# orange-vertex/depthmapX

Hardware: AMD Instinct MI355X
Metric: grid cells/sec for VISPREP makeGraph + VGA global on N×N grid (higher is better)
Workload: dtype f64

## Files before the change

### depthmapx_amd/csrc/api/makegraph.hip

```cpp

typedef void (*mk_kernel_t)(const MakeGraphParams*);
#ifndef DMX_MK_WPE
#define DMX_MK_WPE 5
#endif
#define MKK(PROF, FIXED, COUNT, MAXD, FAR) makegraph_kernel<DMX_MK_WPE, PROF, FIXED, COUNT, MAXD, FAR>
static mk_kernel_t mk_kernel(bool fixed, bool count, bool maxd, bool far) {
    if (count) {
        if (!fixed || maxd) return MKK(false, false, true, false, false);
        return far ? MKK(false, true, true, false, true) : MKK(false, true, true, false, false);
    }
    if (verbose()) {
        if (!fixed || maxd) return MKK(true, false, false, false, false);
        return far ? MKK(true, true, false, false, true) : MKK(true, true, false, false, false);
    }
    if (!fixed) return MKK(false, false, false, false, false);
    if (maxd) return far ? MKK(false, true, false, true, true) : MKK(false, true, false, true, false);
    return far ? MKK(false, true, false, false, true) : MKK(false, true, false, false, false);
}
#undef MKK

static int mk_sqrt_err(dmx_ctx* ctx, long long nmax, double* err) {
    if (ctx->sqrt_err_nmax < nmax) {
        DevBuf<unsigned long long> e;
        HIPCHK(e.alloc(1));
// ... 163 lines not shown
            HIPCHK(hipMemsetAsync(ctx->counters.p + 4, 0, sizeof(int), ctx->stream));
            MakeGraphParams P;
            P.cols = h.cols(); P.rows = h.rows();
            P.spacing = h.spacing(); P.blx = h.bottom_left().x; P.bly = h.bottom_left().y;
            P.maxdist = maxdist;
            P.cellw = pm->d_cellw.p; P.segs = pm->d_segs.p; P.node_cell = pm->d_node_cell.p;
            P.sqrt_err = sqrt_err;
            P.node_begin = node_begin; P.node_end = node_end;
            P.work_counter = ctx->counters.p + 0;
            P.ctl = ctx->d_ctl;
            ctx->h_ctl->progress = 0;
            P.error = ctx->counters.p + 1;
            P.pool_cursor = (unsigned long long*)(ctx->counters.p + 2);
            P.pool_capacity = pool_cap; P.pool = g->pool.p;
            P.node_run_start = g->node_run_start.p; P.bin_nruns = g->bin_nruns.p; P.bin_count = g->bin_count.p;
            P.bin_dist = g->bin_dist.p; P.attrs = g->attrs.p;
            P.stageA = stA.p; P.stageB = stB.p; P.prefix = pref.p; P.runcnt = rcnt.p;
            P.capA = (int)capA; P.capB = (int)capB; P.gcap = gcap; P.bcap = bcap; P.dmax = D;
            P.bspill = bsp.p; P.bspill_flag = bspf.p; P.spill_cap = spill_cap;
            P.stats = ctx->stats.p;
            P.node_list = list_n < 0 ? nullptr : node_list.p;
            P.list_n = list_n < 0 ? 0 : list_n;
            P.fail_list = fail_list.p;
            P.fail_count = ctx->counters.p + 4;
            P.profile = verbose() ? 1 : 0;
            P.exact_moments = exact_pass ? 1 : 0;
            P.src_work = d_work;
            P.openh = openh.p; P.openh_n = openh_n;
            const bool sym_pass = fuse_sym && !sampling;
            P.sym_prefix = sym_pass ? g->sym_prefix.p : nullptr;
            P.sym_diff = sym_pass ? g->sym_diff.p : nullptr;
            P.sym_ho = sym_pass ? g->sym_ho.p : nullptr;
            P.spans = getenv("DMX_MK_NOSPAN") ? 0 : (getenv("DMX_MK_SPAN") ? std::max(1, atoi(getenv("DMX_MK_SPAN"))) : MK_SPAN_MIN);
            HIPCHK(hipEventRecord(ctx->ev0, ctx->stream));
            if (todo > 0) {
                HIPCHK(dP.alloc(1));
                HIPCHK(hipMemcpyAsync(dP.p, &P, sizeof(P), hipMemcpyHostToDevice, ctx->stream));
                hipLaunchKernelGGL(kern, dim3((unsigned)waves), dim3(64), lds, ctx->stream,
                                   (const MakeGraphParams*)dP.p);
                HIPCHK(hipGetLastError());
            }
            HIPCHK(hipEventRecord(ctx->ev1, ctx->stream));
            HIPCHK(wait_progress(ctx, DMX_PHASE_MAKEGRAPH, todo, 1));
            CANCEL_POINT(ctx);
            float ms = 0;
            HIPCHK(hipEventElapsedTime(&ms, ctx->ev0, ctx->ev1));
            kernel_s += ms * 1e-3;
            int hc[5] = {0, 0, 0, 0, 0};
            HIPCHK(copy_sync(ctx->stream, hc, ctx->counters.p, sizeof(hc), hipMemcpyDeviceToHost));
            const int err = hc[1], nfail = hc[4];
            VLOG("makegraph: attempt %d (%lld sources, gcap %d bcap %d spill %d capB %lld, occupancy %d): %.3f s, %d failed, "
                 "err %d\n", attempt, (long long)todo, gcap, bcap, spill_cap, (long long)capB, occ, ms * 1e-3, nfail, err);
            if (err & KERR_BIN_MISMATCH) return fail(DMX_ERR_STATE, "internal: whichbin outside octant");
            if (err & KERR_POOL_CAPACITY) {
                unsigned long long used = 0;
                std::memcpy(&used, &hc[2], 8);
                pool_cap = std::max<int64_t>(pool_cap * 2, (int64_t)used + 1024);
                pool_over = true;
                break;
            }
            if (nfail == 0) break;
            if (!sampling) {
                reruns += nfail;
                std::vector<int64_t> fl((size_t)nfail);
                HIPCHK(copy_sync(ctx->stream, fl.data(), fail_list.p, (size_t)nfail * 8, hipMemcpyDeviceToHost));
                mk_reruns.insert(mk_reruns.end(), fl.begin(), fl.end());
// ... 21 lines not shown
        HIPCHK(hipEventRecord(ctx->ev0, ctx->stream));
        if (n > 0 && !only) {
            hipLaunchKernelGGL(gridconn_kernel, dim3((unsigned)((n + 255) / 256)), dim3(256), 0, ctx->stream, h.rows(),
                               pm->d_node_cell.p + node_begin, n, g->node_run_start.p, g->bin_nruns.p, g->pool.p,
                               g->gridconn.p);
            HIPCHK(hipGetLastError());
            hipLaunchKernelGGL(node_nruns_kernel, dim3((unsigned)((n + 255) / 256)), dim3(256), 0, ctx->stream,
                               g->bin_nruns.p, n, g->node_nruns.p);
            HIPCHK(hipGetLastError());
        }
        HIPCHK(hipEventRecord(ctx->ev1, ctx->stream));
        HIPCHK(hipStreamSynchronize(ctx->stream));
        float ms = 0;
        HIPCHK(hipEventElapsedTime(&ms, ctx->ev0, ctx->ev1));
        kernel_s += ms * 1e-3;
        int hc[4] = {0, 0, 0, 0};
        HIPCHK(copy_sync(ctx->stream, hc, ctx->counters.p, sizeof(hc), hipMemcpyDeviceToHost));
        unsigned long long used = 0;
        std::memcpy(&used, &hc[2], 8);
        unsigned long long st[32];
        HIPCHK(copy_sync(ctx->stream, st, ctx->stats.p, sizeof(st), hipMemcpyDeviceToHost));
        if (verbose()) {
            st[22] += st[26] + st[27] + st[28];
            double tot = (double)st[22];
            for (int i = 8; i < 18; i++) tot += (double)st[i];
            VLOG("makegraph phases (wave clocks): garbage %.1f%%, ranges %.1f%%, candidates %.1f%%, bins %.1f%%, "
                 "moments %.1f%%, run tracking %.1f%%, placement %.1f%%, publish %.1f%%, depth tail %.1f%%, "
                 "octant setup %.1f%% (%.3g total; %llu depth steps, %llu chunks, %llu candidates)\n", 100 * st[8] / tot,
                 100 * st[9] / tot, 100 * st[10] / tot, 100 * st[11] / tot, 100 * st[12] / tot, 100 * st[13] / tot,
                 100 * st[14] / tot, 100 * st[15] / tot, 100 * st[16] / tot, 100 * st[17] / tot, tot, st[2], st[3], st[0]);
            VLOG("makegraph merges: %llu (%llu with one block), %.2f blocks and %.2f gaps a merge\n", st[18], st[19],
                 st[18] ? (double)st[20] / st[18] : 0.0, st[18] ? (double)st[21] / st[18] : 0.0);
            VLOG("makegraph spans: %.1f%% of the clocks; %llu spans over %llu depths (%.1f each), %llu of %llu visible cells "
                 "(%.1f%%)\n", 100 * st[22] / tot, st[23], st[24], st[23] ? (double)st[24] / st[23] : 0.0, st[25], st[1],
                 st[1] ? 100.0 * st[25] / st[1] : 0.0);
            VLOG("makegraph span parts: rows' class ends and open state %.1f%%, gap depth searches %.1f%%, class pieces "
                 "%.1f%%, the rest (setup, examined, sums) %.1f%% of the clocks; %llu row chunks, %llu (chunk, gap) pairs, "
                 "%llu of them with no visible row\n", 100 * st[26] / tot, 100 * st[27] / tot, 100 * st[28] / tot,
                 100 * (st[22] - st[26] - st[27] - st[28]) / tot, st[29], st[30], st[31]);
        }
        ctx->last_stats[0] = (long long)st[0];
        ctx->last_stats[1] = (long long)st[1];
        ctx->last_stats[2] = (long long)used;
        ctx->last_stats[32] = (long long)st[2];
        ctx->last_stats[33] = (long long)st[3];
        ctx->last_stats[34] = (long long)reruns;
        ctx->last_stats[47] = diag_inexact;
        ctx->last_mk_reruns = std::move(mk_reruns);
        ctx->last_mk_s = mk_total_s + kernel_s;
        g->nruns = (int64_t)used;
        if (fuse_sym) { g->sym_fused = true; g->sym_prefix.reset(); }
        VLOG("makegraph: kernels %.3f s, total %.3f s\n", kernel_s, now_s() - t_start);
        *out = g.release();
        return DMX_OK;
    }
    return fail(DMX_ERR_CAPACITY, "makegraph capacities exceeded after retries");
}

int dmx_makegraph(dmx_ctx* ctx, dmx_pointmap* pm, double maxdist, int boundary, int64_t node_begin, int64_t node_end,
                  dmx_graph** out) {
    return makegraph_impl(ctx, pm, maxdist, boundary, node_begin, node_end, nullptr, nullptr, out);
}

using policy::kMkSourceCost;
using policy::kMkChunkCost;

int dmx_makegraph_balance(dmx_ctx* ctx, dmx_pointmap* pm, double maxdist, int boundary, int32_t world, int64_t stride,
                          int64_t* bounds) {
// ... 133 lines not shown
```

### depthmapx_amd/csrc/dmx_api.hip

```cpp
#include <hip/hip_runtime.h>

#include <execinfo.h>
#include <signal.h>
#include <unistd.h>

#include <algorithm>
#include <array>
#include <chrono>
#include <cstdio>
#include <cstring>
#include <map>
#include <memory>
#include <mutex>
#include <string>
#include <thread>
#include <vector>

#include "../../include/dmx.h"
#include "policy.hpp"
#include "host/bsptree.hpp"
#include "host/graphfile.hpp"
#include "host/graphio.hpp"
#include "host/pointmap.hpp"
#include "kernels/makegraph.hip"
// ... 142 lines not shown
struct dmx_ctx {
    int device = 0;
    bool tile_disabled = false;
    hipStream_t stream = nullptr;
    hipEvent_t ev0 = nullptr, ev1 = nullptr;
    int num_cu = 0;
    double last_mk_s = 0, last_vga_s = 0, last_sd_s = 0;
    long long last_sd_stats[3] = {0, 0, 0};
    long long last_sd_extra[2] = {0, 0};
    int last_sd_mode = 0;
    long long phase_cycles[5] = {0, 0, 0, 0, 0};
    DevBuf<int> counters;
    DevBuf<unsigned long long> stats;
    long long last_stats[48] = {};
    std::vector<int64_t> last_mk_reruns;
    DmxCtl* h_ctl = nullptr;
    DmxCtl* d_ctl = nullptr;
    dmx_progress_fn progress = nullptr;
    void* progress_user = nullptr;
    double progress_interval = 0.5;
    hipEvent_t ev_poll = nullptr;
    double last_fill_s[2] = {0, 0};
    double last_iso_bsp_s = 0, last_iso_kernel_s = 0;
    long long last_iso[4] = {0, 0, 0, 0};
    double sqrt_err = 0.0;
    long long sqrt_err_nmax = 0;
    long long last_fill_levels = 0;
};

struct dmx_pointmap {
    std::unique_ptr<PointMapHost> host;
    int uploaded_for = -1;
    uint64_t version = 1, uploaded_version = 0;
    int64_t nnodes = 0;
    std::vector<int32_t> node_cell;
    DevBuf<uint32_t> d_cellw;
    DevBuf<double> d_segs;
    DevBuf<int32_t> d_node_cell;
    DevBuf<int32_t> d_cell_node;
    DevBuf<uint8_t> d_node_flags;
    DevBuf<unsigned long long> d_seed_tiles;
    DevBuf<unsigned long long> d_nonexp_tiles;
};

struct dmx_graph {
    dmx_ctx* ctx = nullptr;
    dmx_pointmap* pm = nullptr;
    std::vector<int32_t> merges;
    bool merges_ready = false;
    DevBuf<int2> d_mpairs;
    DevBuf<int2> d_mamb;
    int nmamb = 0;
    DevBuf<int32_t> d_merge_cell;
    int64_t nnodes = 0, node_begin = 0, node_end = 0;
    int64_t nruns = 0;
    DevBuf<Run> pool;
    DevBuf<int64_t> node_run_start;
    DevBuf<int32_t> node_nruns;
    DevBuf<int32_t> bin_nruns;
    DevBuf<uint16_t> bin_count;
    DevBuf<float> bin_dist;
    DevBuf<float> attrs;
    DevBuf<uint8_t> gridconn;
    DevBuf<unsigned long long> uf_tiles;
    DevBuf<unsigned long long> notuf_tiles;
    int64_t uf_count = -1;
// ... 53 lines not shown
    HIPCHK(hipSetDevice(g->ctx->device));
    const PointMapHost& h = *g->pm->host;
    const int64_t C = h.cells(), m = (int64_t)g->merges.size() / 2;
    const auto& st = h.state();
    const int rows = h.rows();
    auto cf_odd = [&](int32_t c) {
        const int x = c / rows, y = c % rows;
        return (st[c] & CELL_CONTEXTFILLED) && !((x % 2) == 0 && (y % 2) == 0);
    };
    std::vector<int32_t> per_cell((size_t)C, -1);
    std::vector<int2> pairs((size_t)m), amb;
    for (int64_t i = 0; i < m; i++) {
        const int32_t a = g->merges[2 * i], b = g->merges[2 * i + 1];
        if (!(st[a] & CELL_FILLED) || !(st[b] & CELL_FILLED)) return fail(DMX_ERR_ARG, "merge link to a cell without a node");
        per_cell[a] = b;
        per_cell[b] = a;
        pairs[i] = make_int2(a, b);
        if (cf_odd(a) != cf_odd(b)) amb.push_back(cf_odd(a) ? make_int2(a, b) : make_int2(b, a));
    }
    HIPCHK(g->d_mpairs.alloc(m));
    HIPCHK(g->d_merge_cell.alloc(C));
    HIPCHK(hipMemcpyAsync(g->d_mpairs.p, pairs.data(), m * sizeof(int2), hipMemcpyHostToDevice, g->ctx->stream));
    HIPCHK(hipMemcpyAsync(g->d_merge_cell.p, per_cell.data(), C * 4, hipMemcpyHostToDevice, g->ctx->stream));
    g->nmamb = (int)amb.size();
    if (g->nmamb) {
        HIPCHK(g->d_mamb.alloc(amb.size()));
        HIPCHK(hipMemcpyAsync(g->d_mamb.p, amb.data(), amb.size() * sizeof(int2), hipMemcpyHostToDevice, g->ctx->stream));
    }
    HIPCHK(hipStreamSynchronize(g->ctx->stream));
    g->merges_ready = true;
    return DMX_OK;
}

static void clean_distance(const PointMapHost& h, std::vector<uint32_t>& cellw) {
    const int W = h.cols(), H = h.rows();
    std::vector<uint32_t> d((size_t)W * H);
    for (int x = 0; x < W; x++)
        for (int y = 0; y < H; y++) {
            const size_t c = (size_t)x * H + y;
            const bool clean = (cellw[c] & 0xFFu) == 1u;
            d[c] = clean ? (uint32_t)std::min(std::min(x + 1, y + 1), std::min(W - x, H - y)) : 0u;
        }
    for (int x = 0; x < W; x++)
        for (int y = 0; y < H; y++) {
            const size_t c = (size_t)x * H + y;
            uint32_t v = d[c];
            if (!v) continue;
            if (y > 0) v = std::min(v, d[c - 1] + 1);
            if (x > 0) {
                const size_t l = c - H;
                v = std::min(v, d[l] + 1);
                if (y > 0) v = std::min(v, d[l - 1] + 1);
                if (y + 1 < H) v = std::min(v, d[l + 1] + 1);
            }
            d[c] = v;
        }
    for (int x = W - 1; x >= 0; x--)
        for (int y = H - 1; y >= 0; y--) {
            const size_t c = (size_t)x * H + y;
            uint32_t v = d[c];
            if (!v) continue;
            if (y + 1 < H) v = std::min(v, d[c + 1] + 1);
            if (x + 1 < W) {
                const size_t r = c + H;
                v = std::min(v, d[r] + 1);
                if (y > 0) v = std::min(v, d[r - 1] + 1);
                if (y + 1 < H) v = std::min(v, d[r + 1] + 1);
            }
            d[c] = v;
        }
    for (size_t c = 0; c < d.size(); c++)
        if ((cellw[c] & 0xFFu) == 1u) cellw[c] = (std::min(d[c], CELL_DIST_MAX) << 8) | 1u;
}

int upload_pointmap(dmx_ctx* ctx, dmx_pointmap* pm) {
    PointMapHost& h = *pm->host;
    if (!h.lines_blocked()) h.block_lines();
    if (pm->uploaded_version == pm->version && pm->uploaded_for == ctx->device) return DMX_OK;
    if (pm->uploaded_for >= 0 && pm->uploaded_for != ctx->device) {
        pm->d_cellw.reset(); pm->d_segs.reset(); pm->d_node_cell.reset(); pm->d_cell_node.reset();
        pm->d_node_flags.reset(); pm->d_seed_tiles.reset(); pm->d_nonexp_tiles.reset();
        pm->uploaded_for = -1;
    }
    const int64_t C = h.cells();
    std::vector<uint32_t> cellw((size_t)C);
    const auto& st = h.state();
    const auto& off = h.seg_off();
    pm->node_cell.clear();
    std::vector<int32_t> cell_node((size_t)C, -1);
    std::vector<uint8_t> flags;
    for (int64_t c = 0; c < C; c++) {
        const int32_t n = off[c + 1] - off[c];
        if (n > 127) return fail(DMX_ERR_UNSUPPORTED, "more than 127 occluder pieces in one grid cell");
        if ((int64_t)off[c] >= (1 << 24)) return fail(DMX_ERR_UNSUPPORTED, "more than 16M occluder pieces");
        const bool filled = st[c] & CELL_FILLED;
        cellw[c] = pack_cell(filled, (uint32_t)n, (uint32_t)off[c]);
        if (filled) {
            cell_node[c] = (int32_t)pm->node_cell.size();
            pm->node_cell.push_back((int32_t)c);
            flags.push_back((st[c] & CELL_CONTEXTFILLED) ? 1 : 0);
        }
    }
    pm->nnodes = (int64_t)pm->node_cell.size();
    clean_distance(h, cellw);
    const int tw = (h.cols() + 7) / 8, th = (h.rows() + 7) / 8;
    std::vector<unsigned long long> seed((size_t)tw * th, ~0ull), nonexp((size_t)tw * th, 0ull);
    for (int x = 0; x < h.cols(); x++)
        for (int y = 0; y < h.rows(); y++) {
            const int32_t sv = st[h.index(x, y)];
            const unsigned long long bit = 1ull << ((y & 7) * 8 + (x & 7));
            if (sv & CELL_FILLED) seed[(size_t)(y >> 3) * tw + (x >> 3)] &= ~bit;
            if ((sv & CELL_CONTEXTFILLED) && !((x % 2) == 0 && (y % 2) == 0)) nonexp[(size_t)(y >> 3) * tw + (x >> 3)] |= bit;
        }
    HIPCHK(hipSetDevice(ctx->device));
    HIPCHK(pm->d_cellw.alloc(C));
    HIPCHK(pm->d_segs.alloc(std::max<size_t>(h.segs().size(), 4)));
    HIPCHK(pm->d_node_cell.alloc(std::max<int64_t>(pm->nnodes, 1)));
    HIPCHK(pm->d_cell_node.alloc(C));
    HIPCHK(pm->d_node_flags.alloc(std::max<int64_t>(pm->nnodes, 1)));
    HIPCHK(pm->d_seed_tiles.alloc(seed.size()));
    HIPCHK(pm->d_nonexp_tiles.alloc(nonexp.size()));
    HIPCHK(hipMemcpyAsync(pm->d_nonexp_tiles.p, nonexp.data(), nonexp.size() * 8, hipMemcpyHostToDevice, ctx->stream));
    HIPCHK(hipMemcpyAsync(pm->d_cellw.p, cellw.data(), C * 4, hipMemcpyHostToDevice, ctx->stream));
    if (!h.segs().empty())
        HIPCHK(hipMemcpyAsync(pm->d_segs.p, h.segs().data(), h.segs().size() * 8, hipMemcpyHostToDevice, ctx->stream));
    if (pm->nnodes) {
        HIPCHK(hipMemcpyAsync(pm->d_node_cell.p, pm->node_cell.data(), pm->nnodes * 4, hipMemcpyHostToDevice, ctx->stream));
        HIPCHK(hipMemcpyAsync(pm->d_node_flags.p, flags.data(), pm->nnodes, hipMemcpyHostToDevice, ctx->stream));
    }
    HIPCHK(hipMemcpyAsync(pm->d_cell_node.p, cell_node.data(), C * 4, hipMemcpyHostToDevice, ctx->stream));
    HIPCHK(hipMemcpyAsync(pm->d_seed_tiles.p, seed.data(), seed.size() * 8, hipMemcpyHostToDevice, ctx->stream));
    HIPCHK(hipStreamSynchronize(ctx->stream));
    pm->uploaded_version = pm->version;
    pm->uploaded_for = ctx->device;
    return DMX_OK;
}

// ... 213 lines not shown
```

### depthmapx_amd/csrc/kernels/makegraph.hip

```cpp
#include "common.hpp"
#include "span.hpp"


namespace dmx {

#ifndef MK_PFIND
#define MK_PFIND 1
#endif
#ifndef MK_SPAN_CB
#define MK_SPAN_CB 0
#endif
#ifndef MK_SPAN_GSKIP
#define MK_SPAN_GSKIP 1
#endif
#ifndef MK_WFRED
#define MK_WFRED 0
#endif
#ifndef MK_SPAN_RCP
#define MK_SPAN_RCP 0
#endif
#ifndef MK_SPAN_LSUM
#define MK_SPAN_LSUM 1
#endif
constexpr int MK_GCAP0 = 16, MK_BCAP0 = 32;
constexpr int MK_SPAN_MIN = 4;
constexpr int MK_OPEN_LDS = 1024;
constexpr int64_t MK_CAPACITY_TAG = 1ll << 62, MK_NODE_MASK = MK_CAPACITY_TAG - 1;
constexpr uint32_t MK_OPEN_ADJ = 0x80000000u;
constexpr int MK_REC_SHALLOW = 58, MK_REC_DEEP = 59;
constexpr int16_t MK_RUN_FLAG = 0x4000;

struct MakeGraphParams {
    int cols, rows;
    double spacing, blx, bly;
    double maxdist;
    const uint32_t* cellw;
    double sqrt_err;
    const double* segs;
    const int32_t* node_cell;
    int64_t node_begin, node_end;
    int* work_counter;
    DmxCtl* ctl;
    unsigned long long* pool_cursor;
    int64_t pool_capacity;
    Run* pool;
    int64_t* node_run_start;
    int32_t* bin_nruns;
    uint16_t* bin_count;
    float* bin_dist;
    float* attrs;
    unsigned long long* stageA;
    Run* stageB;
    uint32_t* prefix;
    uint32_t* runcnt;
    int capA, capB;
    int gcap, bcap;
    double2* bspill;
    int* bspill_flag;
    int spill_cap;
    int dmax;
    int* error;
    unsigned long long* stats;
    const int64_t* node_list;
    int64_t list_n;
    int64_t* fail_list;
    int* fail_count;
    int profile;
    int exact_moments;
    uint32_t* src_work;
    uint32_t* openh;
    int openh_n;
    const unsigned long long* sym_prefix;
    unsigned long long* sym_diff;
    unsigned long long* sym_ho;
    int spans;
};

#define MK_T(i)                                                           \
    if (PROF) {                                                           \
        const unsigned long long n_ = __builtin_amdgcn_s_memtime();       \
        cyc[i] += n_ - tmark;                                             \
        tmark = n_;                                                       \
    }

__constant__ int c_sector_base[8] = {13, 1, 17, 29, 21, 25, 9, 5};
__constant__ int c_axis_bin[8] = {16, 0, -1, -1, -1, 24, 8, -1};
__constant__ int c_diag_bin[8] = {12, 4, 20, 28, -1, -1, -1, -1};
__constant__ int c_row_asc[8] = {1, 1, 0, 0, 0, 1, 0, 1};
__constant__ int c_d_asc[8] = {0, 1, 0, 1, 0, 0, 1, 1};
__constant__ int c_axis_low[8] = {0, 1, 0, 0, 0, 1, 1, 0};
__constant__ int c_diag_low[8] = {1, 0, 0, 1, 0, 0, 0, 0};
__constant__ int c_seg_order[8] = {1, 7, 6, 0, 2, 4, 5, 3};

__device__ __forceinline__ void octant_cell(int q, int cx, int cy, int depth, int ind, int& hx, int& hy) {
    int x = (q >= 4 ? ind : depth);
    int y = (q >= 4 ? depth : ind);
    hx = (short)(cx + ((q & 1) ? x : -x));
    hy = (short)(cy + ((q <= 1 || q >= 6) ? y : -y));
}

__device__ __forceinline__ double tanify(double cxp, double cyp, double px, double py, int q) {
    switch (q) {
    case 0: return (py - cyp) / (cxp - px);
    case 1: return (py - cyp) / (px - cxp);
    case 2: return (cyp - py) / (cxp - px);
    case 3: return (cyp - py) / (px - cxp);
    case 4: return (cxp - px) / (cyp - py);
    case 5: return (px - cxp) / (cyp - py);
// ... 201 lines not shown
        else if (i - bcap < P.spill_cap) spill[i - bcap] = v;
    };
    auto get_block = [&](int i) -> double2 { return i < bcap ? L.blocks[i] : spill[i - bcap]; };
    auto set_flag = [&](int i, int f) {
        if (i < bcap) L.bflag[i] = f;
        else spill_flag[i - bcap] = f;
    };
    auto get_flag = [&](int i) -> int { return i < bcap ? L.bflag[i] : spill_flag[i - bcap]; };
    auto put_sorted = [&](int i, double2 v) {
        if (i < bcap) L.bsorted[i] = v;
        else spill[P.spill_cap + i - bcap] = v;
    };
    auto get_sorted = [&](int i) -> double2 { return i < bcap ? L.bsorted[i] : spill[P.spill_cap + i - bcap]; };
    auto pref = P.prefix + (size_t)wave_global * (3 * (D + 1) + 4);
    auto rcnt = P.runcnt + (size_t)wave_global * (3 * (D + 1) + 4);
    const double sp = P.spacing;
    const bool symflags = P.sym_diff != nullptr && P.cols < 16384 && P.rows < 16384;

    const int AX = 3 * (D + 1);
    auto openh = P.openh + (size_t)wave_global * P.openh_n;
    const bool far_rows = FIXED ? FAR : (D + 4 > MK_OPEN_LDS);
    auto ld_open = [&](int i) -> uint32_t {
        return (!far_rows || i < MK_OPEN_LDS) ? L.openr[i] : ld_l2(&openh[i - MK_OPEN_LDS]);
    };
    auto st_open = [&](int i, uint32_t v) {
        if (!far_rows || i < MK_OPEN_LDS) L.openr[i] = v;
        else st_l2(&openh[i - MK_OPEN_LDS], v);
    };
    for (int i = lane; i < min(D + 4, MK_OPEN_LDS); i += 64) L.openr[i] = 0;
    __syncthreads();
    unsigned long long cyc[14] = {0, 0, 0, 0, 0, 0, 0, 0, 0, 0, 0, 0, 0, 0};
    unsigned long long mst[4] = {0, 0, 0, 0};
    unsigned long long spst[6] = {0, 0, 0, 0, 0, 0};
    unsigned long long tmark = PROF ? __builtin_amdgcn_s_memtime() : 0;

    for (;;) {
        int s_idx = 0;
        if (lane == 0) s_idx = ctl_poll(P.ctl, atomicAdd(P.work_counter, 1));
        s_idx = __shfl(s_idx, 0);
        int64_t node;
        if (P.node_list) {
            if (s_idx >= P.list_n) break;
            node = P.node_list[s_idx] & MK_NODE_MASK;
        } else {
            node = P.node_begin + s_idx;
            if (node >= P.node_end) break;
        }
        const int cell = P.node_cell[node];
        const int cx = __builtin_amdgcn_readfirstlane(cell / P.rows), cy = __builtin_amdgcn_readfirstlane(cell % P.rows);
        const double c0x = P.blx + sp * 1.0 * (double)cx, c0y = P.bly + sp * 1.0 * (double)cy;
        if (lane < 32) { L.binc[lane] = 0; L.bfar[lane] = 0; L.bnr[lane] = 0; }
        __syncthreads();

        double tsum = 0.0, tsum2 = 0.0;
        double s1 = 0.0, s2 = 0.0;
        unsigned long long s2n = 0;
        int mcnt = 0;
        int nsize = 0;
        unsigned long long examined = 0;
#if MK_SPAN_LSUM
        int nsize_l = 0;
        unsigned long long examined_l = 0;
#endif
        uint32_t nsteps = 0, nchunks = 0;
        int bpos = 0;
        bool failed = false;
// ... 18 lines not shown
            }
            if (lane == 0) { L.misc[0] = 1; L.misc[1] = 0; }
            if (lane == 0) L.gaps[0] = make_double2(0.0, 1.0);
            __syncthreads();
            for (int i = lane; i < own_n; i += 64) {
                const double* sg = P.segs + 4 * (size_t)(own_off + i);
                Seg l = make_seg(Vec2{sg[0], sg[1]}, Vec2{sg[2], sg[3]});
                if (clip_seg(l, vp)) {
                    Vec2 a = l.start(), b = l.end();
                    double ta = tanify(c0x, c0y, a.x, a.y, q), tb = tanify(c0x, c0y, b.x, b.y, q);
                    const int slot = atomicAdd(&L.misc[1], 1);
                    put_block(slot, (ta < tb) ? make_double2(ta - 1e-10, tb + 1e-10) : make_double2(tb - 1e-10, ta + 1e-10));
                }
            }
            __syncthreads();

            int ng = 1;
            int dq = 0;
            int diag_n = 0, diag_min = 0, diag_max = 0;
            int nA = 0;
            const int q_sector = c_sector_base[q], q_axis = c_axis_bin[q], q_diag = c_diag_bin[q];
            unsigned obinp = 0;
            {
                const double rr[5] = {0.0, 0.1, 0.4, 0.8, 1.0};
#pragma unroll
                for (int k = 0; k < 5; k++) {
                    const double mj = 10.0, mn = 10.0 * rr[k];
                    const double ax = (q >= 4 ? mn : mj), ay = (q >= 4 ? mj : mn);
                    obinp |= (unsigned)whichbin((q & 1) ? ax : -ax, (q <= 1 || q >= 6) ? ay : -ay) << (6 * k);
                }
                obinp = __builtin_amdgcn_readfirstlane(obinp);
            }
#define OBIN(k) ((int)__builtin_amdgcn_ubfe(obinp, (unsigned)(6 * (k)), 6u))
            int depth = 0;
            MK_T(9);
            uint32_t pf_w = 0;
#if MK_PFIND
            int pf_ind = 0;
            int2 pf_gc = make_int2(0, -1);
#endif
            bool pf_ok = false;
            int pf_T = 0;
            for (;;) {
                int nb = L.misc[1];
                if (nb > 0) pf_ok = false;
                if (PROF && nb > 0) { mst[0]++; mst[1] += (nb == 1); mst[2] += nb; mst[3] += ng; }
                if (nb > bcap + P.spill_cap) { failed = true; if (lane == 0) atomicOr(P.error, KERR_BLOCK_CAPACITY); }
                if (failed) break;
                if (nb == 1 && ng <= 64) {
                    const double2 kb = L.blocks[0];
                    const double kx = kb.x, ky = kb.y;
                    const bool have = lane < ng;
                    double gx = 0.0, gy = 0.0;
                    if (have) { const double2 v = L.gaps[lane]; gx = v.x; gy = v.y; }
                    double ax = gx, ay = gy, bx2 = 0.0, by2 = 0.0;
                    int nout = have ? 1 : 0;
                    if (have && !(ky < gx)) {
                        bool create = true;
                        double cx_ = gx, cy_ = gy;
                        if (kx <= cx_) { create = false; if (ky > cx_) cx_ = ky; }
                        if (ky >= cy_) { create = false; if (kx < cy_) cy_ = kx; }
                        ax = cx_;
                        ay = cy_;
                        if (cy_ <= cx_ + 1e-10) nout = 0;
                        else if (!(ky > cy_) && create) { nout = 2; ay = kx; bx2 = ky; by2 = cy_; }
                    }
// ... 216 lines not shown
                        }
                        octant_cell(q, cx, cy, depth, ind, hx, hy);
                        ingrid = (hx >= 0 && hx < P.cols && hy >= 0 && hy < P.rows);
                    }
                    int nlb = 0, offb = 0;
                    if (ingrid) {
                        const int hc = hx * P.rows + hy;
                        w = (pf_ok && t0 == 0) ? pf_w : P.cellw[hc];
                        const int nl = cell_nseg(w), off = cell_seg_off(w);
                        const bool centregap = ind >= gcr.x && ind <= gcr.y;
                        if (centregap && cell_filled(w) &&
                            (ind != 0 || q == 0 || q == 1 || q == 5 || q == 6) && (ind != depth || q < 4)) {
                            const double px = P.blx + sp * 1.0 * (double)hx, py = P.bly + sp * 1.0 * (double)hy;
                            bool blocked = false;
                            if (hasmax || nl > 0) {
                                Seg ray = make_seg(Vec2{c0x, c0y}, Vec2{px, py});
                                if (hasmax && ray.length() > P.maxdist) blocked = true;
                                const double tol = sp * 1e-10;
                                for (int k = 0; k < nl && !blocked; k++) {
                                    const double* sg = P.segs + 4 * (size_t)(off + k);
                                    Seg s = make_seg(Vec2{sg[0], sg[1]}, Vec2{sg[2], sg[3]});
                                    if (rects_touch(ray.r, s.r, tol) && segs_cross(ray, s, tol)) blocked = true;
                                }
                            }
                            add = !blocked;
                        }
                        for (int k = 0; k < nl; k++) {
                            const double* sg = P.segs + 4 * (size_t)(off + k);
                            double ta = tanify(c0x, c0y, sg[0], sg[1], q), tb = tanify(c0x, c0y, sg[2], sg[3], q);
                            const int slot = atomicAdd(&L.misc[1], 1);
                            put_block(slot, (ta < tb) ? make_double2(ta - 1e-10, tb + 1e-10) : make_double2(tb - 1e-10, ta + 1e-10));
                        }
                    }
                    if (valid) lmin = min(lmin, ingrid ? cell_span_dist(w) : 0);
                    hasgaps |= (ballot(ingrid) != 0ull);
                    MK_T(2);
                    unsigned long long am = ballot(add);
                    if (am) {
                        int bin = -1;
                        double this_dist = 0.0;
                        {
                            const float fd = (float)depth, fi = (float)ind, mg = 1e-6f * fd;
                            const float e15 = fi - 0.267949192f * fd, e30 = fi - 0.577350269f * fd;
                            int k = 1 + (e15 >= 0.0f) + (e30 >= 0.0f);
                            k = (ind == depth) ? 4 : k;
                            k = (ind == 0) ? 0 : k;
                            bin = OBIN(k);
                            const bool amb = add & (ind != 0) & (ind != depth) & ((fabsf(e15) < mg) | (fabsf(e30) < mg));
                            if (ballot(amb) != 0ull) {
                                if (amb) {
                                    const double px = P.blx + sp * 1.0 * (double)hx, py = P.bly + sp * 1.0 * (double)hy;
                                    bin = whichbin(px - c0x, py - c0y);
                                }
                            }
                        }
                        const unsigned n2 = (unsigned)(depth * depth) + __umul24((unsigned)ind, (unsigned)ind);
                        if (add) {
                            atomicAdd(&L.binc[bin], 1u);
                            atomicMax(&L.bfar[bin], n2);
                        }
                        MK_T(3);
                        if (exact) {
                            if (add) this_dist = sqrt((double)n2) * sp;
                            const int d_lo = __double2loint(this_dist), d_hi = __double2hiint(this_dist);
                            unsigned long long mm = am;
                            while (mm) {
                                const int l = __ffsll((long long)mm) - 1;
// ... 24 lines not shown
                                if ((o & 1u) && oslot == slot && ol == depth - 1) {
                                    st_open(ind, pack_open(slot, os, depth) | (o & MK_OPEN_ADJ));
                                } else {
                                    const bool adj = (o & 1u) && ol == depth - 1;
                                    if (o & 1u) {
                                        emit = true;
                                        rec = pack_emit(oslot, ind, os, ol, 0) | ((unsigned long long)(o >> 31) << MK_REC_SHALLOW) |
                                              ((unsigned long long)adj << MK_REC_DEEP);
                                    }
                                    st_open(ind, pack_open(slot, depth, depth) | (adj ? MK_OPEN_ADJ : 0u));
                                }
                            }
                        }
                        unsigned long long dm = ballot(add && ind == depth && q < 4);
                        if (dm) {
                            if (diag_n == 0) diag_min = depth;
                            diag_max = depth;
                            diag_n++;
                        }
                        unsigned long long em = ballot(emit);
                        if (em) {
                            int pos = nA + prefix_popc(em);
                            if (emit) {
                                if (pos < P.capA) stA[pos] = rec;
                            }
                            nA += __popcll(em);
                        }
                    }
                    MK_T(5);
                }
                if (nA > P.capA) { failed = true; if (lane == 0) atomicOr(P.error, KERR_STAGE_CAPACITY); }
                if (!hasgaps) break;
                dq = depth;
                if (__builtin_expect(spans && !failed && L.misc[1] == 0 && ballot(lmin < span_min + 2) == 0ull, 0)) {
                    int mind = lmin;
#if MK_WFRED
                    mind = __ockl_wfred_min_i32(mind);
#else
                    for (int off = 32; off >= 1; off >>= 1) mind = min(mind, __shfl_xor(mind, off));
#endif
                    const int d0 = depth + 1, d1 = depth + (mind - 2);
                    if (far_rows) __syncthreads(); else wave_sync();
                    SpanOct so;
                    so.q = q; so.cx = cx; so.cy = cy; so.blx = P.blx; so.bly = P.bly; so.sp = sp; so.c0x = c0x; so.c0y = c0y;
                    so.obinp = obinp;
                    const bool axis_row = (q == 0 || q == 1 || q == 5 || q == 6);
                    for (int g = lane; g < ng; g += 64) {
                        const double2 z = L.gaps[g];
#if MK_SPAN_RCP
                        L.gaps2[g] = make_double2(__builtin_amdgcn_rcp(z.x), __builtin_amdgcn_rcp(z.y));
#else
                        L.gaps2[g] = make_double2(1.0 / z.x, 1.0 / z.y);
#endif
                    }
                    wave_sync();
                    const int R0 = max(0, gap_cl(L.gaps[0].x, d0)), R1 = min(d1, gap_ch(L.gaps[ng - 1].y, d1));
                    int nsp = 0;
                    for (int rb = R0; rb <= R1; rb += 64) {
                        if (COUNT || PROF) nchunks++;
                        const int ind = rb + lane;
                        const bool live = ind <= R1;
                        int t3 = ind, t2 = ind;
                        if (live && ind > 0) {
                            const double x3 = (double)ind * 1.7320508075688772, x2 = (double)ind * 3.7320508075688776;
                            t3 = (x3 + 3.0 < (double)d0) ? d0 - 1 : (x3 - 3.0 > (double)d1) ? d1
                                                                  : class_last(so, ind, 3, 0.5773502691896257);
                            t2 = (x2 + 3.0 < (double)d0) ? d0 - 1 : (x2 - 3.0 > (double)d1) ? d1
                                                                  : class_last(so, ind, 2, 0.2679491924311227);
                            t3 = max(t3, ind);
                            t2 = max(t2, t3);
                        }
                        uint32_t o = live ? ld_open(ind) : 0u;
                        bool diag = false;
                        if (PROF) spst[3]++;
                        MK_T(11);
                        for (int g = ng - 1; g >= 0; g--) {
                            const double2 z = L.gaps[g], iz = L.gaps2[g];
                            const double gs_ = z.x, ge_ = z.y;
#if MK_SPAN_GSKIP
                            if (ballot(live && ind >= gap_cl(gs_, d0) && ind <= gap_ch(ge_, d1)) == 0ull) continue;
#endif
                            int p = 1, r = 0;
                            if (live) {
                                int a = (ind == 0) ? d0 : clamp_est(ceil((double)ind * iz.y), d0, d1 + 1);
                                while (a > d0 && gap_ch(ge_, a - 1) >= ind) a--;
                                while (a <= d1 && gap_ch(ge_, a) < ind) a++;
                                int c = (gs_ > 0.0) ? clamp_est(floor((double)ind * iz.x), d0 - 1, d1) : d1;
                                while (c < d1 && gap_cl(gs_, c + 1) <= ind) c++;
                                while (c >= d0 && gap_cl(gs_, c) > ind) c--;
                                if (g > 0) {
                                    const double gp_ = L.gaps[g - 1].y;
                                    int f = clamp_est(floor(((double)ind + 0.5) * L.gaps2[g - 1].y - 0.5), d0 - 1, d1);
                                    const int m = min(ind, d1);
                                    if (f < m) f = m;
                                    while (f < d1 && gap_b(gp_, f + 1) <= ind) f++;
                                    while (f >= d0 && gap_b(gp_, f) > ind) f--;
                                    c = min(c, f);
                                }
                                p = a;
                                r = c;
                                if (ind == 0 && !axis_row) r = p - 1;
                                if (q >= 4 && p <= ind) p = ind + 1;
                            }
                            if (p <= r) {
                                double sa = 0.0, sb = 0.0;
                                const unsigned i2 = (unsigned)(ind * ind);
                                int d = p;
                                for (; d + 1 <= r; d += 2) {
                                    sa += sqrt_nr((double)((unsigned)(d * d) + i2));
                                    sb += sqrt_nr((double)((unsigned)((d + 1) * (d + 1)) + i2));
// ... 38 lines not shown
                                    } else {
                                        const int slot = (cc == 0) ? 3 : bin - q_sector;
                                        const int oslot = (o >> 1) & 3, os = (o >> 3) & 0x3fff, ol = (o >> 17) & 0x3fff;
                                        if ((o & 1u) && oslot == slot && ol == a - 1) {
                                            o = pack_open(slot, os, b) | (o & MK_OPEN_ADJ);
                                        } else {
                                            const bool adj = (o & 1u) && ol == a - 1;
                                            if (o & 1u) {
                                                emit = true;
                                                rec = pack_emit(oslot, ind, os, ol, 0) | ((unsigned long long)(o >> 31) << MK_REC_SHALLOW) |
                                                      ((unsigned long long)adj << MK_REC_DEEP);
                                            }
                                            o = pack_open(slot, a, b) | (adj ? MK_OPEN_ADJ : 0u);
                                        }
                                    }
                                }
                                const unsigned long long em = ballot(emit);
                                if (em) {
                                    const int pos = nA + prefix_popc(em);
                                    if (emit && pos < P.capA) stA[pos] = rec;
                                    nA += __popcll(em);
                                }
                            }
                            MK_T(13);
                        }
                        if (live) st_open(ind, o);
                        const unsigned long long dm = ballot(diag);
                        if (dm) {
                            if (diag_n == 0) diag_min = rb + (__ffsll((long long)dm) - 1);
                            diag_max = rb + 63 - __clzll((long long)dm);
                            diag_n += __popcll(dm);
                        }
                    }
                    unsigned long long exs = 0;
                    for (int db = d0; db <= d1; db += 64) {
                        const int d = db + lane;
                        int F = 0, T = 0;
                        for (int g = 0; g < ng; g++) {
                            const double2 z = L.gaps[g];
                            const int lo = gap_lo(z.x, d), b = min(gap_hi(z.y, d), d), a = max(lo, F);
                            T += (b >= a) ? (b - a + 1) : 0;
                            if (b >= lo) F = max(F, b);
                        }
                        if (d <= d1) exs += (unsigned long long)T;
                    }
#if MK_SPAN_LSUM
                    examined_l += exs;
                    nsize_l += nsp;
                    if (PROF) {
                        for (int off = 32; off >= 1; off >>= 1) nsp += __shfl_xor(nsp, off);
                        spst[0]++; spst[1] += (unsigned long long)(d1 - d0 + 1); spst[2] += (unsigned long long)__shfl(nsp, 0);
                    }
#else
                    for (int off = 32; off >= 1; off >>= 1) {
                        exs += __shfl_xor(exs, off);
                        nsp += __shfl_xor(nsp, off);
                    }
                    examined += __shfl(exs, 0);
                    nsize += __shfl(nsp, 0);
                    if (PROF) { spst[0]++; spst[1] += (unsigned long long)(d1 - d0 + 1); spst[2] += (unsigned long long)__shfl(nsp, 0); }
#endif
                    if (COUNT || PROF) nsteps++;
                    depth = d1;
                    dq = depth;
                    if (nA > P.capA) { failed = true; if (lane == 0) atomicOr(P.error, KERR_STAGE_CAPACITY); }
                    if (far_rows) __syncthreads(); else wave_sync();
                    MK_T(10);
                }
                pf_ok = false;
                if (ng <= 8 && !failed && L.misc[1] == 0) {
                    const int d1 = depth + 1;
                    int F1 = 0, T1 = 0, pind = -1;
                    for (int g = 0; g < ng; g++) {
                        const double2 z = L.gaps[g];
                        const int lo = (int)ceil(z.x * (d1 - 0.5) - 0.5);
                        const int hi = (int)floor(z.y * (d1 + 0.5) + 0.5);
                        const int b = min(hi, d1);
                        const int a = max(lo, F1);
                        const int c = (b >= a) ? (b - a + 1) : 0;
                        const int2 gcg = make_int2((int)ceil(z.x * d1), (int)floor(z.y * d1));
                        if (lane >= T1 && lane < T1 + c) {
                            pind = a + (lane - T1);
#if MK_PFIND
                            pf_gc = gcg;
#endif
                        }
                        if (lane == 0) {
                            L.ga[g] = a;
                            L.gpre[g] = T1;
                            L.gc[g] = gcg;
                        }
                        T1 += c;
                        if (b >= lo) F1 = max(F1, b);
                    }
                    pf_T = T1;
#if MK_PFIND
                    pf_ind = pind;
#endif
                    if (pind >= 0) {
// ... 211 lines not shown
            }
            if (sym) {
                for (int off = 32; off >= 1; off >>= 1) ho += __shfl_xor(ho, off);
                if (lane == 0) P.sym_ho[k] = ho;
            }
            if (lane == 0) P.node_run_start[k] = (int64_t)base;
        }
        __syncthreads();
        if (lane < 32) {
            P.bin_nruns[k * 32 + lane] = L.bnr[lane];
            P.bin_count[k * 32 + lane] = (uint16_t)L.binc[lane];
            const unsigned nf = L.bfar[lane];
            P.bin_dist[k * 32 + lane] = nf ? (float)(sqrt((double)nf) * sp) : 0.0f;
        }
        if (lane == 0) {
            atomicAdd(&P.stats[0], examined);
            atomicAdd(&P.stats[1], (unsigned long long)nsize);
            if (COUNT) {
                atomicAdd(&P.stats[2], (unsigned long long)nsteps);
                atomicAdd(&P.stats[3], (unsigned long long)nchunks);
                P.src_work[2 * k] = nsteps;
                P.src_work[2 * k + 1] = nchunks;
            } else if (PROF) {
                atomicAdd(&P.stats[2], (unsigned long long)nsteps);
                atomicAdd(&P.stats[3], (unsigned long long)nchunks);
                for (int i = 0; i < 4; i++) atomicAdd(&P.stats[18 + i], mst[i]);
            }
            if (PROF) {
                for (int i = 0; i < 10; i++) atomicAdd(&P.stats[8 + i], cyc[i]);
                atomicAdd(&P.stats[22], cyc[10]);
                for (int i = 0; i < 3; i++) atomicAdd(&P.stats[23 + i], spst[i]);
                for (int i = 0; i < 3; i++) atomicAdd(&P.stats[26 + i], cyc[11 + i]);
                for (int i = 0; i < 3; i++) atomicAdd(&P.stats[29 + i], spst[3 + i]);
            }
            P.attrs[k * 3 + 0] = (float)nsize;
            P.attrs[k * 3 + 1] = m1f;
            P.attrs[k * 3 + 2] = m2f;
        }
        __syncthreads();
        for (int i = 0; i < 14; i++) cyc[i] = 0;
        for (int i = 0; i < 4; i++) mst[i] = 0;
        for (int i = 0; i < 6; i++) spst[i] = 0;
        MK_T(7);
    }
}

__global__ void gridconn_kernel(int rows, const int32_t* node_cell, int64_t n, const int64_t* node_run_start,
                                const int32_t* bin_nruns, const Run* pool, uint8_t* out) {
    int64_t k = (int64_t)blockIdx.x * blockDim.x + threadIdx.x;
    if (k >= n) return;
    const int cell = node_cell[k];
    const int cx = cell / rows, cy = cell % rows;
    const int nx[8] = {cx + 1, cx + 1, cx, cx - 1, cx - 1, cx - 1, cx, cx + 1};
    const int ny[8] = {cy, cy + 1, cy + 1, cy + 1, cy, cy - 1, cy - 1, cy - 1};
    int64_t off = node_run_start[k];
    uint8_t gc = 0;
    for (int b = 0; b < 32; b++) {
        const int nr = bin_nruns[k * 32 + b];
        if ((b & 3) == 0) {
            const int i = b >> 2;
            for (int r = 0; r < nr; r++) {
                Run ru = pool[off + r];
                bool hit;
                if (ru.y0 == ru.y1 && ru.x0 != ru.x1) hit = (ny[i] == ru.y0 && nx[i] >= ru.x0 && nx[i] <= ru.x1);
                else if (ru.x0 == ru.x1 && ru.y0 != ru.y1) hit = (nx[i] == ru.x0 && ny[i] >= ru.y0 && ny[i] <= ru.y1);
                else if (ru.x0 == ru.x1) hit = (nx[i] == ru.x0 && ny[i] == ru.y0);
                else {
                    int dy = (ru.y1 > ru.y0) ? 1 : -1;
                    hit = nx[i] >= ru.x0 && nx[i] <= ru.x1 && (ny[i] - ru.y0) == dy * (nx[i] - ru.x0);
                }
                if (hit) { gc |= (uint8_t)(1 << i); break; }
            }
        }
        off += nr;
    }
// ... 5 lines not shown
```

### depthmapx_amd/csrc/kernels/span.hpp

```cpp
#pragma once
#include <cmath>
#include <cstdint>

#if defined(__HIPCC__)
#define DMX_SPAN_HD __host__ __device__
#else
#define DMX_SPAN_HD
#endif

namespace dmx {

DMX_SPAN_HD inline int whichbin(double gx, double gy) {
    int bin;
    double ratio;
    if (!(fabs(gy) > fabs(gx))) {
        ratio = fabs(gy) / fabs(gx);
        if (gx > 0.0) bin = (gy >= 0.0) ? 0 : -32;
        else bin = (gy >= 0.0) ? -16 : 16;
    } else {
        ratio = fabs(gx) / fabs(gy);
        if (gy > 0.0) bin = (gx >= 0.0) ? -8 : 8;
        else bin = (gx >= 0.0) ? 24 : -24;
    }
    if (ratio < 1e-12) {
// ... 83 lines not shown
}

DMX_SPAN_HD inline int gap_lo(double s, int d) { return (int)ceil(s * (d - 0.5) - 0.5); }
DMX_SPAN_HD inline int gap_hi(double e, int d) { return (int)floor(e * (d + 0.5) + 0.5); }
DMX_SPAN_HD inline int gap_b(double e, int d) { const int h = gap_hi(e, d); return h < d ? h : d; }
DMX_SPAN_HD inline int gap_cl(double s, int d) { return (int)ceil(s * d); }
DMX_SPAN_HD inline int gap_ch(double e, int d) { return (int)floor(e * d); }

DMX_SPAN_HD inline int clamp_est(double x, int a, int b) {
    if (!(x >= (double)a)) return a;
    if (x >= (double)b) return b;
    return (int)x;
}

DMX_SPAN_HD inline void span_row_gap(int ind, double s, double e, bool has_prev, double ep, int d0, int d1, int& p, int& r) {
    int a = (ind == 0) ? d0 : clamp_est(ceil((double)ind / e), d0, d1 + 1);
    while (a > d0 && gap_ch(e, a - 1) >= ind) a--;
    while (a <= d1 && gap_ch(e, a) < ind) a++;
    p = a;
    int c = (s > 0.0) ? clamp_est(floor((double)ind / s), d0 - 1, d1) : d1;
    while (c < d1 && gap_cl(s, c + 1) <= ind) c++;
    while (c >= d0 && gap_cl(s, c) > ind) c--;
    r = c;
    if (has_prev) {
        int f = clamp_est(floor(((double)ind + 0.5) / ep - 0.5), d0 - 1, d1);
        const int m = ind < d1 ? ind : d1;
        if (f < m) f = m;
        while (f < d1 && gap_b(ep, f + 1) <= ind) f++;
        while (f >= d0 && gap_b(ep, f) > ind) f--;
        if (f < r) r = f;
    }
}

}
```

Baseline: 148,700.

## Extend span fast path to octants bounded by fully closed grid walls

Detects grid sides that are completely walled and uses them so clean-distance no longer limits cells near a closed boundary. In the makegraph kernel, octants that run toward a closed wall can now take the multi-depth span shortcut. A single open gap whose last block is a wall cell is merged analytically along the wall row, and span depth bounds are clamped to the wall. The aim is to cut per-depth stepping for sources near enclosing walls, which is common in enclosed test grids. This adds considerable branching and numeric validation logic, with a risk of subtle visibility errors.

```diff
diff --git a/depthmapx_amd/csrc/api/makegraph.hip b/depthmapx_amd/csrc/api/makegraph.hip
--- a/depthmapx_amd/csrc/api/makegraph.hip
+++ b/depthmapx_amd/csrc/api/makegraph.hip
@@ -219,6 +219,7 @@
             P.sym_diff = sym_pass ? g->sym_diff.p : nullptr;
             P.sym_ho = sym_pass ? g->sym_ho.p : nullptr;
             P.spans = getenv("DMX_MK_NOSPAN") ? 0 : (getenv("DMX_MK_SPAN") ? std::max(1, atoi(getenv("DMX_MK_SPAN"))) : MK_SPAN_MIN);
+            P.wall = pm->wall_sides;
             HIPCHK(hipEventRecord(ctx->ev0, ctx->stream));
             if (todo > 0) {
                 HIPCHK(dP.alloc(1));
@@ -306,8 +307,9 @@
             VLOG("makegraph merges: %llu (%llu with one block), %.2f blocks and %.2f gaps a merge\n", st[18], st[19],
                  st[18] ? (double)st[20] / st[18] : 0.0, st[18] ? (double)st[21] / st[18] : 0.0);
             VLOG("makegraph spans: %.1f%% of the clocks; %llu spans over %llu depths (%.1f each), %llu of %llu visible cells "
-                 "(%.1f%%)\n", 100 * st[22] / tot, st[23], st[24], st[23] ? (double)st[24] / st[23] : 0.0, st[25], st[1],
-                 st[1] ? 100.0 * st[25] / st[1] : 0.0);
+                 "(%.1f%%); %llu wall spans over %llu depths (closed sides 0x%x)\n", 100 * st[22] / tot, st[23], st[24],
+                 st[23] ? (double)st[24] / st[23] : 0.0, st[25], st[1], st[1] ? 100.0 * st[25] / st[1] : 0.0, st[4], st[5],
+                 (unsigned)pm->wall_sides);
             VLOG("makegraph span parts: rows' class ends and open state %.1f%%, gap depth searches %.1f%%, class pieces "
                  "%.1f%%, the rest (setup, examined, sums) %.1f%% of the clocks; %llu row chunks, %llu (chunk, gap) pairs, "
                  "%llu of them with no visible row\n", 100 * st[26] / tot, 100 * st[27] / tot, 100 * st[28] / tot,
diff --git a/depthmapx_amd/csrc/dmx_api.hip b/depthmapx_amd/csrc/dmx_api.hip
--- a/depthmapx_amd/csrc/dmx_api.hip
+++ b/depthmapx_amd/csrc/dmx_api.hip
@@ -198,6 +198,8 @@
     std::unique_ptr<PointMapHost> host;
     int uploaded_for = -1;
     uint64_t version = 1, uploaded_version = 0;
+    int wall_sides = 0;
+    bool uploaded_nowall = false;
     int64_t nnodes = 0;
     std::vector<int32_t> node_cell;
     DevBuf<uint32_t> d_cellw;
@@ -317,14 +319,22 @@
     return DMX_OK;
 }
 
-static void clean_distance(const PointMapHost& h, std::vector<uint32_t>& cellw) {
+static void clean_distance(const PointMapHost& h, std::vector<uint32_t>& cellw, int sides) {
     const int W = h.cols(), H = h.rows();
     std::vector<uint32_t> d((size_t)W * H);
     for (int x = 0; x < W; x++)
         for (int y = 0; y < H; y++) {
             const size_t c = (size_t)x * H + y;
             const bool clean = (cellw[c] & 0xFFu) == 1u;
-            d[c] = clean ? (uint32_t)std::min(std::min(x + 1, y + 1), std::min(W - x, H - y)) : 0u;
+            const bool online = ((sides & 1) && x == 0) || ((sides & 2) && x == W - 1) || ((sides & 4) && y == 0) ||
+                                ((sides & 8) && y == H - 1);
+            const bool wallc = online && (cellw[c] & 0xFFu) == 2u;
+            uint32_t b = CELL_DIST_MAX;
+            if (!(sides & 1)) b = std::min(b, (uint32_t)(x + 1));
+            if (!(sides & 2)) b = std::min(b, (uint32_t)(W - x));
+            if (!(sides & 4)) b = std::min(b, (uint32_t)(y + 1));
+            if (!(sides & 8)) b = std::min(b, (uint32_t)(H - y));
+            d[c] = (clean || wallc) ? b : 0u;
         }
     for (int x = 0; x < W; x++)
         for (int y = 0; y < H; y++) {
@@ -358,10 +368,25 @@
         if ((cellw[c] & 0xFFu) == 1u) cellw[c] = (std::min(d[c], CELL_DIST_MAX) << 8) | 1u;
 }
 
+static int closed_sides(int W, int H, const std::vector<uint32_t>& cellw) {
+    if (W < 3 || H < 3) return 0;
+    int sides = 15;
+    for (int y = 1; y < H - 1; y++) {
+        if (cellw[(size_t)y] & 1u) sides &= ~1;
+        if (cellw[(size_t)(W - 1) * H + y] & 1u) sides &= ~2;
+    }
+    for (int x = 1; x < W - 1; x++) {
+        if (cellw[(size_t)x * H] & 1u) sides &= ~4;
+        if (cellw[(size_t)x * H + H - 1] & 1u) sides &= ~8;
+    }
+    return sides;
+}
+
 int upload_pointmap(dmx_ctx* ctx, dmx_pointmap* pm) {
     PointMapHost& h = *pm->host;
     if (!h.lines_blocked()) h.block_lines();
-    if (pm->uploaded_version == pm->version && pm->uploaded_for == ctx->device) return DMX_OK;
+    const bool nowall = getenv("DMX_MK_NOWALL") != nullptr;
+    if (pm->uploaded_version == pm->version && pm->uploaded_for == ctx->device && pm->uploaded_nowall == nowall) return DMX_OK;
     if (pm->uploaded_for >= 0 && pm->uploaded_for != ctx->device) {
         pm->d_cellw.reset(); pm->d_segs.reset(); pm->d_node_cell.reset(); pm->d_cell_node.reset();
         pm->d_node_flags.reset(); pm->d_seed_tiles.reset(); pm->d_nonexp_tiles.reset();
@@ -387,7 +412,9 @@
         }
     }
     pm->nnodes = (int64_t)pm->node_cell.size();
-    clean_distance(h, cellw);
+    pm->wall_sides = nowall ? 0 : closed_sides(h.cols(), h.rows(), cellw);
+    pm->uploaded_nowall = nowall;
+    clean_distance(h, cellw, pm->wall_sides);
     const int tw = (h.cols() + 7) / 8, th = (h.rows() + 7) / 8;
     std::vector<unsigned long long> seed((size_t)tw * th, ~0ull), nonexp((size_t)tw * th, 0ull);
     for (int x = 0; x < h.cols(); x++)
diff --git a/depthmapx_amd/csrc/kernels/makegraph.hip b/depthmapx_amd/csrc/kernels/makegraph.hip
--- a/depthmapx_amd/csrc/kernels/makegraph.hip
+++ b/depthmapx_amd/csrc/kernels/makegraph.hip
@@ -24,6 +24,8 @@
 #endif
 constexpr int MK_GCAP0 = 16, MK_BCAP0 = 32;
 constexpr int MK_SPAN_MIN = 4;
+constexpr int MK_NOWALL = 1 << 28;
+constexpr int MK_NOCAND = 1 << 24;
 constexpr int MK_OPEN_LDS = 1024;
 constexpr int64_t MK_CAPACITY_TAG = 1ll << 62, MK_NODE_MASK = MK_CAPACITY_TAG - 1;
 constexpr uint32_t MK_OPEN_ADJ = 0x80000000u;
@@ -74,6 +76,7 @@
     unsigned long long* sym_diff;
     unsigned long long* sym_ho;
     int spans;
+    int wall;
 };
 
 #define MK_T(i)                                                           \
@@ -341,6 +344,7 @@
     unsigned long long cyc[14] = {0, 0, 0, 0, 0, 0, 0, 0, 0, 0, 0, 0, 0, 0};
     unsigned long long mst[4] = {0, 0, 0, 0};
     unsigned long long spst[6] = {0, 0, 0, 0, 0, 0};
+    unsigned long long wsp[2] = {0, 0};
     unsigned long long tmark = PROF ? __builtin_amdgcn_s_memtime() : 0;
 
     for (;;) {
@@ -425,6 +429,13 @@
                 obinp = __builtin_amdgcn_readfirstlane(obinp);
             }
 #define OBIN(k) ((int)__builtin_amdgcn_ubfe(obinp, (unsigned)(6 * (k)), 6u))
+            int Bq = MK_NOWALL;
+            {
+                const int bside = (q < 4) ? (q <= 1 ? 8 : 4) : ((q & 1) ? 2 : 1);
+                const int bdist = (q < 4) ? (q <= 1 ? P.rows - 1 - cy : cy) : ((q & 1) ? P.cols - 1 - cx : cx);
+                if (P.wall & bside) Bq = bdist;
+                Bq = __builtin_amdgcn_readfirstlane(Bq);
+            }
             int depth = 0;
             MK_T(9);
             uint32_t pf_w = 0;
@@ -707,7 +718,10 @@
                             put_block(slot, (ta < tb) ? make_double2(ta - 1e-10, tb + 1e-10) : make_double2(tb - 1e-10, ta + 1e-10));
                         }
                     }
-                    if (valid) lmin = min(lmin, ingrid ? cell_span_dist(w) : 0);
+                    if (valid) {
+                        const bool wallc = ind >= Bq && (!ingrid || (w & 0xFFu) == 2u);
+                        lmin = min(lmin, wallc ? MK_NOCAND : ingrid ? cell_span_dist(w) : 0);
+                    }
                     hasgaps |= (ballot(ingrid) != 0ull);
                     MK_T(2);
                     unsigned long long am = ballot(add);
@@ -798,14 +812,86 @@
                 if (nA > P.capA) { failed = true; if (lane == 0) atomicOr(P.error, KERR_STAGE_CAPACITY); }
                 if (!hasgaps) break;
                 dq = depth;
-                if (__builtin_expect(spans && !failed && L.misc[1] == 0 && ballot(lmin < span_min + 2) == 0ull, 0)) {
+                if (__builtin_expect(spans && !failed && L.misc[1] <= (Bq < MK_NOWALL ? 1 : 0) && ballot(lmin < span_min + 2) == 0ull, 0)) {
                     int mind = lmin;
 #if MK_WFRED
                     mind = __ockl_wfred_min_i32(mind);
 #else
                     for (int off = 32; off >= 1; off >>= 1) mind = min(mind, __shfl_xor(mind, off));
 #endif
-                    const int d0 = depth + 1, d1 = depth + (mind - 2);
+                    int Aq = MK_NOWALL;
+                    {
+                        const int aside = (q < 4) ? ((q & 1) ? 2 : 1) : (q >= 6 ? 8 : 4);
+                        const int adist = (q < 4) ? ((q & 1) ? P.cols - 1 - cx : cx) : (q >= 6 ? P.rows - 1 - cy : cy);
+                        if (P.wall & aside) Aq = adist;
+                    }
+                    const bool wallmode = L.misc[1] != 0;
+                    const int d0 = depth + 1;
+                    int d1 = min(depth + (min(mind, 1 << 20) - 2), Aq - 2);
+                    unsigned long long exs = 0;
+                    double wall_e = 0.0;
+                    if (wallmode) {
+                        const int la = L.ga[ng - 1], lb = la + (L.gpre[ng] - L.gpre[ng - 1]) - 1;
+                        bool degen = false;
+                        for (int g = lane; g < ng - 1; g += 64) {
+                            const double2 z = L.gaps[g];
+                            degen |= !(z.y > z.x + 1e-10);
+                        }
+                        if (!(la <= Bq - 1 && lb >= Bq) || ballot(degen) != 0ull) d1 = depth;
+                        const double gs_ = L.gaps[ng - 1].x;
+                        double Ec = L.gaps[ng - 1].y;
+                        for (int jb = depth; jb <= d1; jb += 64) {
+                            const int j = jb + lane;
+                            const bool act = j <= d1;
+                            double kx = INFINITY, ky = INFINITY;
+                            bool ok = false;
+                            if (act) {
+                                int hx, hy;
+                                octant_cell(q, cx, cy, j, Bq, hx, hy);
+                                if (hx >= 0 && hx < P.cols && hy >= 0 && hy < P.rows) {
+                                    const uint32_t w = P.cellw[hx * P.rows + hy];
+                                    if ((w & 0xFFu) == 2u) {
+                                        const double* sg = P.segs + 4 * (size_t)cell_seg_off(w);
+                                        const double ta = tanify(c0x, c0y, sg[0], sg[1], q), tb = tanify(c0x, c0y, sg[2], sg[3], q);
+                                        kx = (ta < tb) ? ta - 1e-10 : tb - 1e-10;
+                                        ky = (ta < tb) ? tb + 1e-10 : ta + 1e-10;
+                                        ok = true;
+                                    }
+                                }
+                            }
+                            double Ei = kx;
+                            for (int o = 1; o < 64; o <<= 1) {
+                                const double t = __shfl_up(Ei, o);
+                                if (lane >= o && t < Ei) Ei = t;
+                            }
+                            double Ep = __shfl_up(Ei, 1);
+                            if (lane == 0 || Ec < Ep) Ep = Ec;
+                            if (Ec < Ei) Ei = Ec;
+                            ok = ok && wall_merge_ok(gs_, Ep, Ei, kx, ky);
+                            int T = 0;
+                            if (j > depth) {
+                                const double Eu = Ep <= 1.0 ? Ep : 1.0;
+                                int F = 0, nl = 0;
+                                for (int g = 0; g < ng - 1; g++) {
+                                    const double2 z = L.gaps[g];
+                                    const int lo = gap_lo(z.x, j), b = min(gap_hi(z.y, j), j), a = max(lo, F);
+                                    T += (b >= a) ? (b - a + 1) : 0;
+                                    if (b >= lo) F = max(F, b);
+                                }
+                                ok = wall_visit_ok(gs_, Eu, F, j, Bq, nl) && ok;
+                                T += nl;
+                            }
+                            const unsigned long long fm = ballot(act && !ok);
+                            const int nok = fm ? (__ffsll((long long)fm) - 1) : min(64, d1 - jb + 1);
+                            if (lane < nok) exs += (unsigned long long)T;
+                            if (nok > 0) Ec = __shfl(Ei, nok - 1);
+                            if (fm) { d1 = jb + nok - 1; break; }
+                        }
+                        wall_e = Ec;
+                    } else if (Bq < MK_NOWALL) {
+                        d1 = wall_below_last(L.gaps[ng - 1].y, Bq, d0, d1);
+                    }
+                  if (d1 - d0 + 1 >= span_min) {
                     if (far_rows) __syncthreads(); else wave_sync();
                     SpanOct so;
                     so.q = q; so.cx = cx; so.cy = cy; so.blx = P.blx; so.bly = P.bly; so.sp = sp; so.c0x = c0x; so.c0y = c0y;
@@ -820,7 +906,7 @@
 #endif
                     }
                     wave_sync();
-                    const int R0 = max(0, gap_cl(L.gaps[0].x, d0)), R1 = min(d1, gap_ch(L.gaps[ng - 1].y, d1));
+                    const int R0 = max(0, gap_cl(L.gaps[0].x, d0)), R1 = min(d1, wallmode ? Bq - 1 : gap_ch(L.gaps[ng - 1].y, d1));
                     int nsp = 0;
                     for (int rb = R0; rb <= R1; rb += 64) {
                         if (COUNT || PROF) nchunks++;
@@ -841,7 +927,8 @@
                         if (PROF) spst[3]++;
                         MK_T(11);
                         for (int g = ng - 1; g >= 0; g--) {
-                            const double2 z = L.gaps[g], iz = L.gaps2[g];
+                            double2 z = L.gaps[g], iz = L.gaps2[g];
+                            if (wallmode && g == ng - 1) { z.y = 1.0; iz.y = 1.0; }
                             const double gs_ = z.x, ge_ = z.y;
 #if MK_SPAN_GSKIP
                             if (ballot(live && ind >= gap_cl(gs_, d0) && ind <= gap_ch(ge_, d1)) == 0ull) continue;
@@ -946,8 +1033,7 @@
                             diag_n += __popcll(dm);
                         }
                     }
-                    unsigned long long exs = 0;
-                    for (int db = d0; db <= d1; db += 64) {
+                    for (int db = d0; db <= d1 && !wallmode; db += 64) {
                         const int d = db + lane;
                         int F = 0, T = 0;
                         for (int g = 0; g < ng; g++) {
@@ -975,10 +1061,15 @@
                     if (PROF) { spst[0]++; spst[1] += (unsigned long long)(d1 - d0 + 1); spst[2] += (unsigned long long)__shfl(nsp, 0); }
 #endif
                     if (COUNT || PROF) nsteps++;
+                    if (wallmode) {
+                        if (lane == 0) { L.gaps[ng - 1].y = wall_e; L.misc[1] = 0; }
+                        if (PROF) { wsp[0]++; wsp[1] += (unsigned long long)(d1 - d0 + 1); }
+                    }
                     depth = d1;
                     dq = depth;
                     if (nA > P.capA) { failed = true; if (lane == 0) atomicOr(P.error, KERR_STAGE_CAPACITY); }
                     if (far_rows) __syncthreads(); else wave_sync();
+                  }
                     MK_T(10);
                 }
                 pf_ok = false;
@@ -1256,6 +1347,7 @@
                 for (int i = 0; i < 3; i++) atomicAdd(&P.stats[23 + i], spst[i]);
                 for (int i = 0; i < 3; i++) atomicAdd(&P.stats[26 + i], cyc[11 + i]);
                 for (int i = 0; i < 3; i++) atomicAdd(&P.stats[29 + i], spst[3 + i]);
+                for (int i = 0; i < 2; i++) atomicAdd(&P.stats[4 + i], wsp[i]);
             }
             P.attrs[k * 3 + 0] = (float)nsize;
             P.attrs[k * 3 + 1] = m1f;
@@ -1265,6 +1357,7 @@
         for (int i = 0; i < 14; i++) cyc[i] = 0;
         for (int i = 0; i < 4; i++) mst[i] = 0;
         for (int i = 0; i < 6; i++) spst[i] = 0;
+        wsp[0] = wsp[1] = 0;
         MK_T(7);
     }
 }
diff --git a/depthmapx_amd/csrc/kernels/span.hpp b/depthmapx_amd/csrc/kernels/span.hpp
--- a/depthmapx_amd/csrc/kernels/span.hpp
+++ b/depthmapx_amd/csrc/kernels/span.hpp
@@ -139,4 +139,22 @@
     }
 }
 
+
+DMX_SPAN_HD inline bool wall_merge_ok(double s, double ep, double ei, double kx, double ky) {
+    return kx > s + 1e-10 && ky >= ep && ei > s + 1e-10;
 }
+DMX_SPAN_HD inline bool wall_visit_ok(double s, double ep, int F, int j, int B, int& n) {
+    const int lo = gap_lo(s, j), b = gap_b(ep, j), a = lo > F ? lo : F;
+    n = b - a + 1;
+    return F <= B - 1 && a <= B && b >= B && gap_ch(ep, j) >= B - 1;
+}
+DMX_SPAN_HD inline int wall_below_last(double e, int B, int d0, int d1) {
+    int c = clamp_est(floor(((double)B - 0.5) / e - 0.5), d0 - 1, d1);
+    const int m = B - 1 < d1 ? B - 1 : d1;
+    if (c < m) c = m;
+    while (c < d1 && gap_b(e, c + 1) <= B - 1) c++;
+    while (c >= d0 && gap_b(e, c) > B - 1) c--;
+    return c;
+}
+
+}
```

Result: faster. 155,700, median of 6 (+4.7%).
